# hasindu2008/sigtk

Hardware: AMD Instinct MI355X
Metric: event_raw_samples_per_sec (higher is better)
Workload: dtype f32+f64; 1 GPU; sigtk event (DNA params) on 10000 synthetic reads x 100000 samples per GPU (BASELINE configs[1]), device-resident; reads_per_gpu=10000, samples_per_read=100000, samples_per_gpu=1000000000, fallback_reads=0, rerun_chunks=0, long_detector_replays=66843, long_detector_replay_indices=87526, split_reads=0, batches_in_flight=1, parallelism=reads sharded across ranks, no collective

## Files before the change

sigtk_amd/csrc/event_detect.h:

```cpp
#pragma once
#include <utility>

#include "event_device.h"

namespace sgk {

template <int W1>
struct LzCfg {
    static constexpr int W2 = 2 * W1;
    static constexpr int R = 16;
    static constexpr int NP = (W1 == 3) ? 8 : 16;
    static constexpr int NA = (W1 == 3) ? 4 : 8;
    static constexpr int NL = (W1 == 3) ? 8 : 16;
    static constexpr int H1 = W1 / 2;
};
static_assert(LzCfg<3>::NP >= 8 && LzCfg<7>::NP >= 16, "prefix ring holds P(i) .. P(i+W2+1)");

#ifndef SGK_EVENT_LEAD
#define SGK_EVENT_LEAD 1
#endif

constexpr int LZ_NONE = -(1 << 29);
constexpr int LZ_NREC = 8;
constexpr int LZ_RING_WORDS = 16;

struct LzSnap {
    LzSnapState init[64];
    LzSnapState at_e[64];
    LzSnapState st0[64];
};
__device__ inline bool lz_equal(const LzSnapState &a, const LzSnapState &b) {
    return a.sp == b.sp && __float_as_int(a.sv) == __float_as_int(b.sv) && a.lm == b.lm && a.r0 == b.r0 &&
           a.bits == b.bits;
}
struct LzLds {
    uint32_t ring[64][LZ_RING_WORDS + 1];
    LzSnap snap;
    LzRun runs[64][LZ_NREC];
    int nrec[64];
};

template <typename T>
__device__ __attribute__((noinline)) float tstat_exact_at(const T *base, Scale sc, int i, int w) {
    double A = 0.0, A2 = 0.0, B = 0.0, B2 = 0.0;
    for (int k = 0; k < w; ++k) {
        const float xa = to_pa(base[i - w + k], sc);
        const float xb = to_pa(base[i + k], sc);
        A = A + (double)xa;
        A2 = A2 + (double)(xa * xa);
        B = B + (double)xb;
        B2 = B2 + (double)(xb * xb);
    }
    if (w == 3) return sgk_tstat_ref<3>(A, A2, B, B2);
    if (w == 6) return sgk_tstat_ref<6>(A, A2, B, B2);
    if (w == 7) return sgk_tstat_ref<7>(A, A2, B, B2);
    return sgk_tstat_ref<14>(A, A2, B, B2);
}

template <typename T>
struct Lead16;
template <>
struct Lead16<int16_t> {
    uint32_t w[8];
    template <int U>
    __device__ __forceinline__ float get(const Scale &sc) const {
        const int v = (U & 1) ? ((int)w[U / 2] >> 16) : (int)(short)(w[U / 2] & 0xffffu);
        const float shifted = (float)v + sc.offf;
        return shifted * sc.unit;
    }
};
template <>
struct Lead16<float> {
    float w[16];
    template <int U>
    __device__ __forceinline__ float get(const Scale &) const { return w[U]; }
};
typedef uint32_t sgk_u32x4_a4 __attribute__((ext_vector_type(4), aligned(4)));

template <typename T>
__device__ __attribute__((noinline)) Lead16<T> lead_fix_head(Lead16<T> g, int pos, T first) {
    T tmp[16];
    __builtin_memcpy(tmp, g.w, sizeof(tmp));
#pragma unroll
    for (int k = 0; k < 16; ++k) tmp[k] = (pos + k < 0) ? first : tmp[k];
    __builtin_memcpy(g.w, tmp, sizeof(tmp));
    return g;
}

constexpr int REP_MAX_EVENTS = 32;
struct RepairCtx {
    const double *P, *P2;
    const int *ev;
    int nev;
    bool all_dirty;
};

__device__ __attribute__((noinline)) float tstat_prefix_at(const double *P, const double *P2, int i, int w) {
    const double p0 = P[i], q0 = P2[i];
    const double A = p0 - P[i - w], A2 = q0 - P2[i - w], B = P[i + w] - p0, B2 = P2[i + w] - q0;
    if (w == 3) return sgk_tstat_ref<3>(A, A2, B, B2);
    if (w == 6) return sgk_tstat_ref<6>(A, A2, B, B2);
    if (w == 7) return sgk_tstat_ref<7>(A, A2, B, B2);
    return sgk_tstat_ref<14>(A, A2, B, B2);
}

template <int W1>
__device__ __forceinline__ void repair_mark(const RepairCtx &rep, int &next_t, int q0, unsigned cnt1, unsigned cnt2,
                                            unsigned &bad1, unsigned &bad2) {
    constexpr int W2 = 2 * W1;
    if (rep.all_dirty) {
#pragma unroll
        for (int u = 0; u < 4; ++u) {
            if ((unsigned)(q0 + u - W1) < cnt1) bad1 |= 1u << u;
            if ((unsigned)(q0 + u - W2) < cnt2) bad2 |= 1u << u;
        }
        return;
    }
    if (next_t > q0 + 3 + W2 - 1) return;
    int nt = 0x7fffffff;
    for (int k = 0; k < rep.nev; ++k) {
        const int t = rep.ev[k];
#pragma unroll
        for (int u = 0; u < 4; ++u) {
            const int i = q0 + u;
            if ((unsigned)(i - t + W1 - 1) < (unsigned)(2 * W1) && (unsigned)(i - W1) < cnt1) bad1 |= 1u << u;
            if ((unsigned)(i - t + W2 - 1) < (unsigned)(2 * W2) && (unsigned)(i - W2) < cnt2) bad2 |= 1u << u;
        }
        if (t + W2 >= q0 + 4 && t < nt) nt = t;
    }
    next_t = nt;
}

constexpr int LZ_PRE = LZ_RING_WORDS;
__device__ __attribute__((noinline)) void lz_emit_slow(uint32_t *ring, unsigned long long *bm, int flushed,
                                                       int i_begin, int s, int e, int p, int cur) {
    const int own_lo = s - i_begin;
    if (p < own_lo) {
        if (cur >= own_lo) ring[LZ_PRE] = (uint32_t)(i_begin + p);
        return;
    }
    if (p >= flushed) {
        atomicOr(&ring[(p >> 5) & (LZ_RING_WORDS - 1)], 1u << (p & 31));
    } else {
        const int pa = i_begin + p;
        if (pa >= s && pa < e) atomicOr(reinterpret_cast<uint32_t *>(bm) + (pa >> 5), 1u << (pa & 31));
    }
}
__device__ __attribute__((noinline)) int lz_record(LzRun *runs, int nrec, int a, int b, int s, int e, int n) {
    if ((b >= s && b < e) || (b == n && e == n && s < n)) {
        if (nrec < LZ_NREC) {
            runs[nrec].a = a;
            runs[nrec].b = b;
        }
        ++nrec;
    }
    return nrec;
}

struct Redo4 {
    float v[4];
};
template <int W1, typename T, bool FLAGGED>
__device__ __attribute__((noinline)) Redo4 redo_quad(const T *base, Scale sc, const double *P, const double *P2, int i0,
                                                     unsigned cnt1, unsigned bits, float t0, float t1, float t2,
                                                     float t3) {
    Redo4 r;
    r.v[0] = t0; r.v[1] = t1; r.v[2] = t2; r.v[3] = t3;
#pragma unroll
    for (int k = 0; k < 4; ++k) {
        if ((bits >> k) & 1u) {
            const int i = i0 + k;
            float v = 0.0f;
            if ((unsigned)(i - W1) < cnt1) {
                if constexpr (FLAGGED) v = tstat_prefix_at(P, P2, i, W1);
                else v = tstat_exact_at<T>(base, sc, i, W1);
            }
            r.v[k] = v;
        }
    }
    return r;
}

typedef unsigned long long lmask_t;
__device__ __forceinline__ bool lane_of(lmask_t m) { return __builtin_amdgcn_inverse_ballot_w64(m); }

template <int W1, typename T, bool FLAGGED, bool LEAD = false>
struct LazyPass {
    static_assert(!(LEAD && FLAGGED), "the fallback keeps its domain checks and TwoSum form");
    using C = LzCfg<W1>;
    static constexpr int W2 = C::W2, R = C::R, NP = C::NP, NA = C::NA, NL = C::NL, H1 = C::H1;
    static constexpr int NA2 = LEAD ? 2 * NA : NA;
    static constexpr int NS = LEAD ? NA : 1;
    static_assert(NA2 > (LEAD ? 2 : 1) * W1 && (!LEAD || NS > W1) && R % NA2 == 0, "ring depths");
    double Ps[NP], Pq[NP];
    SgkARole ar[NA2];
    float ss[NS], sqs[NS];
    SgkLSide ls[NL];
    float t1[4];
    lmask_t nk[4];
    lmask_t hc[4];
    Lead16<T> cur;
    float sv;
    int sp;
    lmask_t inpk, val, strong;
    lmask_t hist[H1 + 1];
    uint32_t bw;
    int lm, r0;
    lmask_t hot;
    int nrec;
    uint32_t *ring;
    LzRun *runs;
    const T *base;
    int lo, hi;
    Scale sc;
    int n, s, e, i_begin, ib, jb, flushed;
    unsigned cnt1, cnt2;
    lmask_t done;
    bool slow;
    bool oldpeak;
    unsigned long long *bm;
    RepairCtx rep;
    int next_t;
    int dirty;

    __device__ __forceinline__ void load_lead(Lead16<T> &dst, int pos) const {
        int p = pos > hi - 16 ? hi - 16 : pos;
        p = p < lo ? lo : p;
        constexpr int NV = 16 * (int)sizeof(T) / 16;
        const sgk_u32x4_a4 *src = reinterpret_cast<const sgk_u32x4_a4 *>(base + p);
        sgk_u32x4_a4 v[NV];
#pragma unroll
        for (int k = 0; k < NV; ++k) v[k] = src[k];
        __builtin_memcpy(dst.w, v, sizeof(dst.w));
        if (pos < 0) dst = lead_fix_head<T>(dst, pos, base[0]);
    }

    template <int U>
    __device__ __forceinline__ void tstep() {
        const float xn = cur.template get<U>(sc);
        const float xqn = xn * xn;
        Ps[(U + W2 + 1) % NP] = Ps[(U + W2) % NP] + (double)xn;
        Pq[(U + W2 + 1) % NP] = Pq[(U + W2) % NP] + (double)xqn;
        if constexpr (LEAD) {
            const double c = Ps[(U + W2) % NP] - Ps[(U + W1) % NP], cq = Pq[(U + W2) % NP] - Pq[(U + W1) % NP];
            const float s_p = (float)c, sq_p = (float)cq;
            const float s_i = ss[U % NS], sq_i = sqs[U % NS];
            ss[(U + W1) % NS] = s_p;
            sqs[(U + W1) % NS] = sq_p;
            bool cv_ok, tail_ok;
            t1[U & 3] = sgk_tstat_try_ab<W1>(s_i, sq_i, ar[(U + NA2 - W1) % NA2], cv_ok, tail_ok);
            nk[U & 3] = ~(__ballot(cv_ok) & __ballot(tail_ok));
            ar[(U + W1) % NA2] = sgk_arole<W1, true>(c, cq);
            const SgkLSide lb = sgk_lside_halves<W2>(s_i, sq_i, s_p, sq_p);
            hc[U & 3] = ~__ballot(sgk_long_cold<W2>(ls[(U + NL - W2) % NL], lb));
            ls[U % NL] = lb;
            return;
        }
        const double p0 = Ps[U % NP], q0 = Pq[U % NP];
        const double b1 = Ps[(U + W1) % NP] - p0, b1q = Pq[(U + W1) % NP] - q0;
        const double b2 = Ps[(U + W2) % NP] - p0, b2q = Pq[(U + W2) % NP] - q0;
        const SgkLSide lb = sgk_lside<W2>(b2, b2q);
        if constexpr (!FLAGGED) {
            bool cv_ok, tail_ok;
            t1[U & 3] = sgk_tstat_try_ab<W1>(b1, b1q, ar[(U + NA - W1) % NA], cv_ok, tail_ok);
            nk[U & 3] = ~(__ballot(cv_ok) & __ballot(tail_ok));
            ar[U % NA] = sgk_arole<W1, true>(b1, b1q);
            hc[U & 3] = ~__ballot(sgk_long_cold<W2>(ls[(U + NL - W2) % NL], lb));
            ls[U % NL] = lb;
        } else {
            bool ok;
            const float v = sgk_tstat_try_ab<W1>(b1, b1q, ar[(U + NA - W1) % NA], ok);
            ok = ok && sgk_try_domain<W1>(b1, b1q, ar[(U + NA - W1) % NA]);
            const double a_s = Ps[(U + W2) % NP], b_s = (double)xn, r_s = Ps[(U + W2 + 1) % NP];
            const double a_q = Pq[(U + W2) % NP], b_q = (double)xqn, r_q = Pq[(U + W2 + 1) % NP];
            const double t_s = r_s - a_s, t_q = r_q - a_q;
            const double e_s = (a_s - (r_s - t_s)) + (b_s - t_s), e_q = (a_q - (r_q - t_q)) + (b_q - t_q);
            const bool clean = U > dirty;
            if (e_s != 0.0 || e_q != 0.0) dirty = dirty > U + 2 * W2 ? dirty : U + 2 * W2;
            ok = ok && clean;
            ar[U % NA] = sgk_arole<W1, false>(b1, b1q);
            bool cold = sgk_long_cold<W2>(ls[(U + NL - W2) % NL], lb);
            cold = cold && clean && sgk_lside_domain(ls[(U + NL - W2) % NL]) && sgk_lside_domain(lb);
            ls[U % NL] = lb;
            t1[U & 3] = v;
            nk[U & 3] = ~__ballot(ok);
            hc[U & 3] = ~__ballot(cold);
        }
    }

    template <bool SLOW>
    __device__ __forceinline__ void dstep_core(const int u, const float v, const lmask_t hck, const lmask_t live) {
        constexpr float ph = DetParam<W1>::ph, thr1 = DetParam<W1>::thr1;
        const float d1 = v - sv;
        const float ee = lane_of(inpk) ? d1 : -d1;
        lmask_t P = __ballot(ee > 0.0f);
        lmask_t Q = __ballot(ee < -ph);
        const lmask_t Tt = __ballot(v > thr1);
        if constexpr (SLOW) {
            P &= live;
            Q &= live;
        }
        const lmask_t ent = Q & ~inpk;
        const lmask_t pos = (inpk & P) | ent;
        strong = (pos & Tt) | (strong & ~pos);
        lmask_t dom = inpk & strong;
        if constexpr (SLOW) dom &= live;
        val = inpk & (val | (Q & strong));
        lmask_t recent = hist[0];
#pragma unroll
        for (int k = 1; k < H1; ++k) recent |= hist[k];
        lmask_t em = val & ~P & ~recent;
        if constexpr (SLOW) em &= live;
        const lmask_t upd = P | ent | em;
        const uint32_t bit = 1u << ((jb + u - H1 - 1) & 31);
        if (SLOW && oldpeak) {
            if (lane_of(em)) {
                lz_emit_slow(ring, bm, flushed, i_begin, s, e, jb + sp, jb + u);
                lm = sp;
                r0 = u;
            }
        } else {
            if (lane_of(em)) {
                bw |= bit;
                lm = sp;
                r0 = u;
            }
            const lmask_t erare = em & ~hist[H1];
            if (erare != 0ull) {
                if (lane_of(erare)) {
                    bw &= ~bit;
                    const int p = jb + sp, own = s - i_begin;
                    if (p >= own) atomicOr(&ring[(p >> 5) & (LZ_RING_WORDS - 1)], 1u << (p & 31));
                    else if (jb >= own) ring[LZ_PRE] = (uint32_t)(i_begin + p);
                }
            }
        }
        sv = lane_of(upd) ? v : sv;
        sp = lane_of(pos) ? u : sp;
        inpk = (inpk & ~em) | ent;
        val = val & ~em;
        if constexpr (SLOW) {
#pragma unroll
            for (int k = H1; k >= 1; --k) hist[k] = (hist[k - 1] & live) | (hist[k] & ~live);
            hist[0] = pos | (hist[0] & ~live);
        } else {
#pragma unroll
            for (int k = H1; k >= 1; --k) hist[k] = hist[k - 1];
            hist[0] = pos;
        }
        const lmask_t rec = dom & hot;
        if (rec != 0ull) {
            if (lane_of(rec)) nrec = lz_record(runs, nrec, ib + max(r0, lm + W1 + 1), ib + u, s, e, n);
        }
        lmask_t on = __ballot(lm < u - W1);
        if constexpr (SLOW) on &= live;
        hot = (hot & ~dom) | (on & hck & (~dom | em));
    }
    __device__ __forceinline__ void bw_advance() {
        const int p = jb - 1;
        atomicOr(&ring[(p >> 5) & (LZ_RING_WORDS - 1)], bw);
        bw = 0u;
    }
    template <int U>
    __device__ __forceinline__ void dstep() {
        if constexpr (U == H1 + 1) {
            if ((jb & 16) == 0) bw_advance();
        }
        dstep_core<false>(U, t1[U & 3], hc[U & 3], ~0ull);
    }
    template <int U>
    __device__ __forceinline__ void dstep_edge() {
        if constexpr (U == H1 + 1) {
            if ((jb & 16) == 0) bw_advance();
        }
        const lmask_t live = ~done & __ballot((unsigned)(ib + U) < (unsigned)n);
        dstep_core<true>(U, t1[U & 3], hc[U & 3], live);
    }
    __device__ __forceinline__ void slow_fix(const int u0) {
#pragma unroll
        for (int k = 0; k < 4; ++k) {
            const bool in1 = (unsigned)(ib + u0 + k - W1) < cnt1;
            t1[k] = in1 ? t1[k] : 0.0f;
            nk[k] &= __ballot(in1);
            hc[k] &= __ballot((unsigned)(ib + u0 + k - W2) < cnt2);
        }
    }

    template <int U0>
    __device__ __forceinline__ void quad() {
        tstep<U0>();
        tstep<U0 + 1>();
        tstep<U0 + 2>();
        tstep<U0 + 3>();
        if (slow) slow_fix(U0);
        if constexpr (FLAGGED) {
            unsigned bad1 = 0u, bad2 = 0u;
            repair_mark<W1>(rep, next_t, ib + U0, cnt1, cnt2, bad1, bad2);
#pragma unroll
            for (int k = 0; k < 4; ++k) {
                nk[k] |= __ballot(((bad1 >> k) & 1u) != 0u);
                hc[k] |= __ballot(((bad2 >> k) & 1u) != 0u);
            }
        }
        const lmask_t anybad = (nk[0] | nk[1] | nk[2] | nk[3]) & ~done;
        if (anybad != 0ull) {
            if (lane_of(anybad)) {
                const unsigned bits = (lane_of(nk[0]) ? 1u : 0u) | (lane_of(nk[1]) ? 2u : 0u) |
                                      (lane_of(nk[2]) ? 4u : 0u) | (lane_of(nk[3]) ? 8u : 0u);
                const Redo4 r4 = redo_quad<W1, T, FLAGGED>(base, sc, rep.P, rep.P2, ib + U0, cnt1, bits, t1[0], t1[1],
                                                           t1[2], t1[3]);
                t1[0] = r4.v[0]; t1[1] = r4.v[1]; t1[2] = r4.v[2]; t1[3] = r4.v[3];
            }
        }
        if (slow) {
            dstep_edge<U0>();
            dstep_edge<U0 + 1>();
            dstep_edge<U0 + 2>();
            dstep_edge<U0 + 3>();
        } else {
            dstep<U0>();
            dstep<U0 + 1>();
            dstep<U0 + 2>();
            dstep<U0 + 3>();
        }
    }

    template <int K>
    __device__ __forceinline__ void init_step(double &ps, double &pq, const float (&w)[2 * W2], double (&hs)[W2 + 1],
                                              double (&hq)[W2 + 1]) {
        const float x = w[K];
        ps = ps + (double)x;
        pq = pq + (double)(x * x);
        constexpr int k1 = K + 1;
        if constexpr (k1 <= W2) { hs[k1] = ps; hq[k1] = pq; }
        if constexpr (k1 >= W2) { Ps[(k1 - W2) % NP] = ps; Pq[(k1 - W2) % NP] = pq; }
        if constexpr (k1 >= W2 && k1 < W2 + W1) {
            constexpr int pr = k1 - W1;
            ar[((k1 - W1 - W2) % NA + NA) % NA] = sgk_arole<W1, !FLAGGED>(ps - hs[pr], pq - hq[pr]);
        }
        if constexpr (k1 >= W2 && k1 < 2 * W2) {
            constexpr int pr = k1 - W2;
            ls[((k1 - 2 * W2) % NL + NL) % NL] = sgk_lside<W2>(ps - hs[pr], pq - hq[pr]);
        }
    }
    template <int... Ks>
    __device__ __forceinline__ void init_rings(const float (&w)[2 * W2], std::integer_sequence<int, Ks...>) {
        double ps = 0.0, pq = 0.0;
        double hs[W2 + 1], hq[W2 + 1];
        hs[0] = 0.0;
        hq[0] = 0.0;
        (init_step<Ks>(ps, pq, w, hs, hq), ...);
    }

    __device__ __forceinline__ void init_lead(const float (&w)[2 * W2]) {
        double hs[2 * W2 + 1], hq[2 * W2 + 1];
        hs[0] = 0.0;
        hq[0] = 0.0;
#pragma unroll
        for (int k = 0; k < 2 * W2; ++k) {
            hs[k + 1] = hs[k] + (double)w[k];
            hq[k + 1] = hq[k] + (double)(w[k] * w[k]);
        }
#pragma unroll
        for (int k = W2; k <= 2 * W2; ++k) { Ps[(k - W2) % NP] = hs[k]; Pq[(k - W2) % NP] = hq[k]; }
        float sf[W2 + W1], sqf[W2 + W1];
#pragma unroll
        for (int j = 0; j < W2 + W1; ++j) {
            const double c = hs[j + W1] - hs[j], cq = hq[j + W1] - hq[j];
            sf[j] = (float)c;
            sqf[j] = (float)cq;
            if (j >= W1) ar[(j - W2 + NA2) % NA2] = sgk_arole<W1, true>(c, cq);
            if (j >= W2) { ss[(j - W2) % NS] = sf[j]; sqs[(j - W2) % NS] = sqf[j]; }
        }
#pragma unroll
        for (int j = 0; j < W2; ++j) ls[(j - W2 + NL) % NL] = sgk_lside_halves<W2>(sf[j], sqf[j], sf[j + W1], sqf[j + W1]);
    }

    template <int... Qs>
    __device__ __forceinline__ void block(std::integer_sequence<int, Qs...>) {
        (quad<4 * Qs>(), ...);
    }
};

__device__ __forceinline__ void lz_flush(uint32_t *ring, unsigned long long *bm, int i_begin, int p0, int own_lo,
                                         int own_hi) {
    uint16_t *bm16 = reinterpret_cast<uint16_t *>(bm);
#pragma unroll
    for (int k = 0; k < 8; ++k) {
        const int p = p0 + 32 * k;
        const int wi = (p >> 5) & (LZ_RING_WORDS - 1);
        const uint32_t w = ring[wi];
        ring[wi] = 0u;
        if (p >= own_lo && p < own_hi) bm16[(i_begin + p) >> 4] = (uint16_t)(w & 0xffffu);
        if (p + 16 >= own_lo && p + 16 < own_hi) bm16[(i_begin + p + 16) >> 4] = (uint16_t)(w >> 16);
    }
}

template <int W1, typename T, bool FLAGGED, bool LEAD = false>
__device__ __forceinline__ void pass_lazy(const ReadCtx<T> &rc, bool given, int lead, int steps, bool active, int s,
                                          int e, LzLds *L, const RepairCtx *rep, bool by_progress = false) {
    using LP = LazyPass<W1, T, FLAGGED, LEAD>;
    constexpr int W2 = LP::W2, R = LP::R;
    if (!__any(active)) return;
    const int l = lane_id();
    LP f;
    f.n = (int)rc.n;
    f.s = active ? s : 0x7fffffff;
    f.e = active ? e : 0x7fffffff;
    f.bm = rc.bm;
    f.sc = rc.sc;
    f.base = rc.base;
    f.lo = (int)(rc.lo < -(1 << 30) ? -(1 << 30) : rc.lo);
    f.hi = (int)(rc.hi > 0x7fffffffLL ? 0x7fffffffLL : rc.hi);
    f.ring = L->ring[l];
    f.runs = L->runs[l];
    const int n = f.n;
    const int i_begin = s - lead;
    f.i_begin = i_begin;
#pragma unroll
    for (int k = 0; k < LZ_RING_WORDS; ++k) f.ring[k] = 0u;
    if (active) f.ring[LZ_PRE] = 0xffffffffu;
#pragma unroll
    for (int k = 0; k < 4; ++k) { f.t1[k] = 0.0f; f.nk[k] = 0ull; f.hc[k] = 0ull; }
    {
        float w[2 * W2];
#pragma unroll
        for (int k = 0; k < 2 * W2; ++k) {
            int p = i_begin - W2 + k;
            p = p > f.hi - 1 ? f.hi - 1 : p;
            p = p < 0 ? 0 : p;
            w[k] = to_pa(f.base[p], f.sc);
        }
#pragma unroll
        for (int k = 0; k < LP::NP; ++k) { f.Ps[k] = 0.0; f.Pq[k] = 0.0; }
        if constexpr (LEAD) f.init_lead(w);
        else f.init_rings(w, std::make_integer_sequence<int, 2 * W2>{});
        if (i_begin == 0) {
            if constexpr (LEAD) {
#pragma unroll
                for (int k = 1; k <= W1; ++k) f.ar[LP::NA2 - k].va = __builtin_nan("");
            } else {
#pragma unroll
                for (int k = 0; k < LP::NA; ++k) f.ar[k].va = __builtin_nan("");
            }
        }
    }
    f.load_lead(f.cur, i_begin + W2);

    f.sv = FLT_MAX;
    f.sp = 0;
    f.inpk = 0ull; f.val = 0ull; f.strong = 0ull; f.hot = 0ull;
#pragma unroll
    for (int k = 0; k <= LP::H1; ++k) f.hist[k] = 0ull;
    f.bw = 0u;
    f.lm = LZ_NONE;
    f.r0 = 0;
    if (__any(given)) {
        LzSnapState st = L->snap.st0[l];
        if (!given) { st.sp = -1; st.sv = FLT_MAX; st.lm = LZ_NONE; st.r0 = i_begin; st.bits = 0u; }
        f.sv = st.sv;
        f.inpk = __ballot((st.bits & 1u) != 0u);
        f.val = __ballot((st.bits & 2u) != 0u);
        f.strong = __ballot((st.bits & 4u) != 0u);
        f.hot = __ballot((st.bits & 8u) != 0u);
        f.sp = (st.bits & 1u) ? st.sp - i_begin : 0;
        f.lm = st.lm == LZ_NONE ? LZ_NONE : st.lm - W1 - i_begin;
#pragma unroll
        for (int k = 0; k <= LP::H1; ++k) f.hist[k] = __ballot((st.bits & 1u) && st.sp == i_begin - 1 - k);
        f.r0 = st.r0 - i_begin;
    }
    f.nrec = 0;
    f.done = ~__ballot(active);
    f.flushed = 0;
    if constexpr (FLAGGED) {
        f.dirty = 2 * W2;
        f.rep = *rep;
        f.next_t = 0x7fffffff;
        for (int k = 0; k < f.rep.nev; ++k) {
            const int t = f.rep.ev[k];
            if (t + W2 >= i_begin && t < f.next_t) f.next_t = t;
        }
    }
    const int main_steps = steps;
    f.cnt1 = (n - 2 * W1 + 1) > 0 ? (unsigned)(n - 2 * W1 + 1) : 0u;
    f.cnt2 = (n - 2 * W2 + 1) > 0 ? (unsigned)(n - 2 * W2 + 1) : 0u;
    const int own_lo = lead, own_hi = active ? lead + (e - s) : lead;

    auto snapshot = [&](int ib) -> LzSnapState {
        LzSnapState st;
        const bool ip = lane_of(f.inpk);
        st.sv = f.sv;
        st.sp = ip ? ib + f.sp : -1;
        st.lm = (f.lm + W1 < 0) ? LZ_NONE : ib + f.lm + W1;
        st.r0 = ib + max(f.r0, f.lm + W1 + 1);
        st.bits = (ip ? 1u : 0u) | ((ip && lane_of(f.val)) ? 2u : 0u) | ((ip && lane_of(f.strong)) ? 4u : 0u) |
                  (lane_of(f.hot) ? 8u : 0u);
        return st;
    };

    constexpr int PRIO_STEPS = 400;
    const int q1 = by_progress ? main_steps - 3 * PRIO_STEPS : -1, q2 = by_progress ? main_steps - 2 * PRIO_STEPS : -1,
              q3 = by_progress ? main_steps - PRIO_STEPS : -1;
    if (by_progress) {
        if (q1 > 0) __builtin_amdgcn_s_setprio(3);
        else if (q2 > 0) __builtin_amdgcn_s_setprio(2);
        else if (q3 > 0) __builtin_amdgcn_s_setprio(1);
        else __builtin_amdgcn_s_setprio(0);
    }
    int jb = 0;
    for (;;) {
        const int ib = i_begin + jb;
        if ((jb & 255) == 0 && jb >= 512) {
            lz_flush(f.ring, f.bm, i_begin, jb - 512, own_lo, own_hi);
            f.flushed = jb - 256;
        }
        const bool lane_edge = ib + R - 1 > n - W2;
        const lmask_t old_peak = __ballot(f.sp < -(256 - 2 * R)) | (__ballot(f.sp + jb < own_lo) & __ballot(jb == own_lo));
        f.oldpeak = (old_peak & f.inpk & ~f.done) != 0ull;
        f.slow = f.oldpeak || (__ballot(lane_edge) & ~f.done) != 0ull;
        f.ib = ib;
        f.jb = jb;
        Lead16<T> nxt;
        f.load_lead(nxt, ib + R + W2);
        f.block(std::make_integer_sequence<int, R / 4>{});
        f.cur = nxt;
        f.sp -= R;
        f.lm = f.lm < LZ_NONE ? LZ_NONE : f.lm - R;
        f.r0 -= R;
        if constexpr (FLAGGED) f.dirty = f.dirty < -(1 << 20) ? f.dirty : f.dirty - R;
        jb += R;
        if (jb == q1) __builtin_amdgcn_s_setprio(2);
        else if (jb == q2) __builtin_amdgcn_s_setprio(1);
        else if (jb == q3) __builtin_amdgcn_s_setprio(0);
        {
            const int nb = i_begin + jb;
            if (active && lead > 0 && jb == lead) L->snap.init[l] = snapshot(nb);
            if (active && nb == e) L->snap.at_e[l] = snapshot(nb);
            const lmask_t reach = __ballot(nb >= e) & ~f.done;
            if ((reach & f.hot) != 0ull) {
                if (lane_of(reach & f.hot) && e == n) f.nrec = lz_record(f.runs, f.nrec, nb + max(f.r0, f.lm + W1 + 1), n, s, e, n);
            }
            f.done |= reach;
            f.inpk &= ~reach;
            f.val &= ~reach;
            f.strong &= ~reach;
        }
        if (jb >= main_steps && f.done == ~0ull) break;
    }
    {
        const int p = jb - LP::H1 - 2 < 0 ? 0 : jb - LP::H1 - 2;
        atomicOr(&f.ring[(p >> 5) & (LZ_RING_WORDS - 1)], f.bw);
    }
    for (int p0 = f.flushed; p0 < jb; p0 += 256) lz_flush(f.ring, f.bm, i_begin, p0, own_lo, own_hi);
    if (active) L->nrec[l] = f.nrec;
}

template <int W1, typename T, bool FLAGGED, bool COLLECT = false>
__device__ inline void replay_run(const ReadCtx<T> &rc, const RepairCtx *rep, bool has, int i, int b, int bits_lo,
                           int bits_hi, EvHeader *hdr, int *found = nullptr) {
    if (has && b > i) atomicAdd(&hdr->n_replay_idx, (unsigned long long)(b - i));
    constexpr int W2 = 2 * W1;
    constexpr float ph = DetParam<W1>::ph, thr2 = DetParam<W1>::thr2;
    const int n = (int)rc.n;
    const unsigned cnt2 = (n - 2 * W2 + 1) > 0 ? (unsigned)(n - 2 * W2 + 1) : 0u;
    uint32_t *bm32 = reinterpret_cast<uint32_t *>(rc.bm);
    int lp = -1;
    float lv = FLT_MAX;
    bool lvalid = false;
    while (__any(has && i < b)) {
        if (has && i < b) {
            float v2 = 0.0f;
            if ((unsigned)(i - W2) < cnt2) {
                if constexpr (FLAGGED) v2 = tstat_prefix_at(rep->P, rep->P2, i, W2);
                else v2 = tstat_exact_at<T>(rc.base, rc.sc, i, W2);
            }
            if (lp < 0) {
                if (v2 < lv) {
                    lv = v2;
                } else if (v2 - lv > ph) {
                    lv = v2;
                    lp = i;
                }
            } else {
                if (v2 > lv) {
                    lv = v2;
                    lp = i;
                }
                if (lv - v2 > ph && lv > thr2) lvalid = true;
                if (lvalid && (i - lp) > W2 / 2) {
                    if (lp > 0 && lp < n && lp >= bits_lo && lp < bits_hi) {
                        if constexpr (COLLECT) *found = 1;
                        else atomicOr(&bm32[lp >> 5], 1u << (lp & 31));
                    }
                    lp = -1;
                    lv = v2;
                    lvalid = false;
                }
            }
            ++i;
        }
    }
}
template <int W1, typename T, bool FLAGGED>
__device__ void replay_long_runs(const ReadCtx<T> &rc, LzLds *L, const RepairCtx *rep, bool active, int bits_lo,
                                 EvHeader *hdr) {
    const int l = lane_id();
    const int nrec = active ? L->nrec[l] : 0;
    for (int k = 0; k < LZ_NREC; ++k) {
        const bool has = k < nrec;
        if (!__any(has)) break;
        const int i = has ? L->runs[l][k].a : 0;
        const int b = has ? L->runs[l][k].b : 0;
        replay_run<W1, T, FLAGGED>(rc, rep, has, i, b, bits_lo, 0x7fffffff, hdr);
    }
}

template <int W1, typename T, bool FLAGGED, bool MULTI = false, bool LEAD = false>
__device__ __forceinline__ int detect_span(const ReadCtx<T> &rc, EvHeader *hdr, LzLds *L, const RepairCtx *rep,
                                           const int a, const int b, const int mode, const int lead_override,
                                           SegState *seg, const int lanes = 64) {
    const int n = (int)rc.n;
    if constexpr (!MULTI) {
        if (b <= a) return 0;
    }
    const int len = b - a;
    int lead = len < 32768 ? LEAD_DNA_SHORT : LEAD_DNA;
    if (W1 == 7) lead = len <= 32768 ? LEAD_RNA_SHORT : LEAD_RNA;
    if constexpr (MULTI) {
        const long long len64 = (long long)len * (64 / lanes);
        lead = len64 < 32768 ? LEAD_DNA_SHORT : LEAD_DNA;
        if (W1 == 7) lead = len64 <= 32768 ? LEAD_RNA_SHORT : LEAD_RNA;
    }
    if (lead_override > 0) lead = lead_override;
    const bool no_fast = (reinterpret_cast<uintptr_t>(rc.base) & 3u) != 0 || rc.hi < (int64_t)n + 16;
    if constexpr (!MULTI) {
        if (no_fast) return 1;
    }
    const int c = MULTI ? (lane_id() & (lanes - 1)) : lane_id();
    int K, s, e0, lead_c;
    if (mode == 1) {
        K = 16 * ((len + 1023) / 1024);
        s = a + c * K;
        e0 = s + K;
        lead_c = lead;
    } else {
        K = MULTI ? chunk_len_lanes(len, lead, lanes) : chunk_len_fast(len, lead);
        s = c == 0 ? a : a + c * K + lead;
        e0 = c == 0 ? a + lead + K : s + K;
        lead_c = c > 0 ? lead : 0;
    }
    int TT = lead + K;
    int Kmax = K;
    if constexpr (MULTI) {
#pragma unroll
        for (int d = 32; d >= 1; d >>= 1) {
            const int o = __shfl_xor(Kmax, d, 64), t = __shfl_xor(TT, d, 64);
            Kmax = o > Kmax ? o : Kmax;
            TT = t > TT ? t : TT;
        }
    }
    const int e = e0 < b ? e0 : b;
    const bool active = s < b && !(MULTI && no_fast);
    {
        LzSnapState z;
        z.sp = -1; z.sv = FLT_MAX; z.lm = LZ_NONE; z.r0 = 0; z.bits = 0u;
        L->snap.init[lane_id()] = z;
        L->snap.at_e[lane_id()] = z;
        L->nrec[lane_id()] = 0;
        L->ring[lane_id()][LZ_PRE] = 0xffffffffu;
    }
    bool run = active;
    bool first = true;
    const int l = lane_id();
    const uint32_t pol = FLAGGED ? 0u : prio_policy(rc.dev);
    for (int iter = 0; iter < 66; ++iter) {
        pass_lazy<W1, T, FLAGGED, LEAD>(rc, first ? (mode == 2 && c == 0) : true, first ? lead_c : 0, first ? TT : Kmax, run,
                                        s, e, L, rep, first && (pol == 1u || pol == 2u));
        __syncthreads();
        const LzSnapState pe = L->snap.at_e[c > 0 ? l - 1 : l];
        const LzSnapState mine = L->snap.init[l];
        const bool bad = active && c > 0 && !lz_equal(pe, mine);
        const unsigned long long badmask = __ballot(bad);
        if (badmask == 0ull) break;
        __syncthreads();
        if (bad) {
            L->snap.init[l] = pe;
            L->snap.st0[l] = pe;
        }
        run = bad;
        first = false;
        if (l == 0) atomicAdd(&hdr->n_rerun, (uint32_t)__popcll(badmask));
        __syncthreads();
    }
    int rcode = 0;
    if constexpr (MULTI) {
        const unsigned long long over = __ballot(active && L->nrec[l] > LZ_NREC);
        const unsigned long long grp = (lanes >= 64 ? ~0ull : ((1ull << lanes) - 1ull)) << (l & ~(lanes - 1));
        if (no_fast) rcode = 1;
        else if (over & grp) rcode = 2;
    } else {
        if (__any(active && L->nrec[l] > LZ_NREC)) return 2;
    }
    const bool mine_ok = active && rcode == 0;
    if (seg) {
        const int last = __popcll(__ballot(active)) - 1;
        if (l == 0) {
            seg->init0 = L->snap.init[0];
            seg->end = L->snap.at_e[last];
        }
        const int nrec = active ? L->nrec[l] : 0;
        int ncross = 0;
        for (int k = 0; k < nrec; ++k) ncross += (L->runs[l][k].a < a) ? 1 : 0;
        const int incl = wave_incl_scan_i(ncross);
        const int total = wave_last_i(incl);
        if (total > SEG_CROSS_MAX) rcode = 2;
        else {
            int at = incl - ncross;
            for (int k = 0; k < nrec; ++k) {
                if (L->runs[l][k].a < a) seg->cross[at++] = L->runs[l][k];
            }
        }
        if (l == 0) seg->n_cross = total > SEG_CROSS_MAX ? 0u : (uint32_t)total;
    }
    const int pre = mine_ok ? (int)L->ring[l][LZ_PRE] : -1;
    const bool pre_out = pre >= 0 && pre < a;
    if (seg) {
        const int npre = pre_out ? 1 : 0;
        const int incl = wave_incl_scan_i(npre);
        const int total = wave_last_i(incl);
        if (total > SEG_PRE_MAX) rcode = 2;
        else if (npre) seg->pre[incl - 1] = pre;
        if (l == 0) seg->n_pre = total > SEG_PRE_MAX ? 0u : (uint32_t)total;
    }
    const unsigned long long hotm = __ballot(mine_ok && L->nrec[l] > 0);
    const bool anypre = __any(pre >= 0);
    if (hotm != 0ull || anypre) {
        if (l == 0 && hotm != 0ull) atomicAdd(&hdr->n_hot_runs, (uint32_t)__popcll(hotm));
        __threadfence_block();
        __syncthreads();
        if (pre >= 0 && !pre_out) atomicOr(reinterpret_cast<uint32_t *>(rc.bm) + (pre >> 5), 1u << (pre & 31));
        if (hotm != 0ull) replay_long_runs<W1, T, FLAGGED>(rc, L, rep, mine_ok, a, hdr);
    }
    return rcode;
}
template <int W1, typename T, bool FLAGGED>
__device__ __forceinline__ int detect_read_lazy(const ReadCtx<T> &rc, EvHeader *hdr, LzLds *L, const RepairCtx *rep) {
    const int n = (int)rc.n;
    if (n <= 0) return 0;
    return detect_span<W1, T, FLAGGED>(rc, hdr, L, rep, 0, n, 0, 0, nullptr);
}

}
```

Before: 301.3 billion samples/s.

## Track run-start bookkeeping with wave bitmasks instead of per-step ballot on lm

```diff
diff --git a/sigtk_amd/csrc/event_detect.h b/sigtk_amd/csrc/event_detect.h
--- a/sigtk_amd/csrc/event_detect.h
+++ b/sigtk_amd/csrc/event_detect.h
@@ -20,6 +20,10 @@
 #define SGK_EVENT_LEAD 1
 #endif
 
+#ifndef SGK_EVENT_BOOK
+#define SGK_EVENT_BOOK 1
+#endif
+
 constexpr int LZ_NONE = -(1 << 29);
 constexpr int LZ_NREC = 8;
 constexpr int LZ_RING_WORDS = 16;
@@ -192,6 +196,8 @@
     static constexpr int NA2 = LEAD ? 2 * NA : NA;
     static constexpr int NS = LEAD ? NA : 1;
     static_assert(NA2 > (LEAD ? 2 : 1) * W1 && (!LEAD || NS > W1) && R % NA2 == 0, "ring depths");
+    static constexpr bool BOOK = ((SGK_EVENT_BOOK) & (FLAGGED ? 4 : (LEAD ? 1 : 2))) != 0;
+    static constexpr int NM = W1 - H1;
     double Ps[NP], Pq[NP];
     SgkARole ar[NA2];
     float ss[NS], sqs[NS];
@@ -206,6 +212,8 @@
     lmask_t hist[H1 + 1];
     uint32_t bw;
     int lm, r0;
+    lmask_t moff[NM - 1];
+    int rs;
     lmask_t hot;
     int nrec;
     uint32_t *ring;
@@ -313,17 +321,37 @@
         if constexpr (SLOW) em &= live;
         const lmask_t upd = P | ent | em;
         const uint32_t bit = 1u << ((jb + u - H1 - 1) & 31);
+        lmask_t off = 0ull, nx[NM - 1];
         if (SLOW && oldpeak) {
             if (lane_of(em)) {
                 lz_emit_slow(ring, bm, flushed, i_begin, s, e, jb + sp, jb + u);
-                lm = sp;
-                r0 = u;
+                if constexpr (BOOK) {
+                    rs = max(u, sp + W1 + 1);
+                } else {
+                    lm = sp;
+                    r0 = u;
+                }
+            }
+            if constexpr (BOOK) {
+                off = moff[0];
+#pragma unroll
+                for (int k = 0; k < NM - 1; ++k) nx[k] = k + 1 < NM - 1 ? moff[k + 1] : 0ull;
+                book_mask_from_sp<NM - 1>(em, u, off, nx);
             }
         } else {
-            if (lane_of(em)) {
-                bw |= bit;
-                lm = sp;
-                r0 = u;
+            if constexpr (BOOK) {
+                if (lane_of(em)) bw |= bit;
+                rs = lane_of(em) ? u + NM : rs;
+                const lmask_t eusual = em & hist[H1];
+                off = moff[0] | eusual;
+#pragma unroll
+                for (int k = 0; k < NM - 1; ++k) nx[k] = k + 1 < NM - 1 ? (moff[k + 1] | eusual) : eusual;
+            } else {
+                if (lane_of(em)) {
+                    bw |= bit;
+                    lm = sp;
+                    r0 = u;
+                }
             }
             const lmask_t erare = em & ~hist[H1];
             if (erare != 0ull) {
@@ -332,7 +360,9 @@
                     const int p = jb + sp, own = s - i_begin;
                     if (p >= own) atomicOr(&ring[(p >> 5) & (LZ_RING_WORDS - 1)], 1u << (p & 31));
                     else if (jb >= own) ring[LZ_PRE] = (uint32_t)(i_begin + p);
+                    if constexpr (BOOK) rs = max(u, sp + W1 + 1);
                 }
+                if constexpr (BOOK) book_mask_from_sp<NM - 2>(erare, u, off, nx);
             }
         }
         sv = lane_of(upd) ? v : sv;
@@ -350,11 +380,31 @@
         }
         const lmask_t rec = dom & hot;
         if (rec != 0ull) {
-            if (lane_of(rec)) nrec = lz_record(runs, nrec, ib + max(r0, lm + W1 + 1), ib + u, s, e, n);
-        }
-        lmask_t on = __ballot(lm < u - W1);
+            if (lane_of(rec)) nrec = lz_record(runs, nrec, ib + run_start(), ib + u, s, e, n);
+        }
+        lmask_t on;
+        if constexpr (BOOK) {
+            on = ~off;
+#pragma unroll
+            for (int k = 0; k < NM - 1; ++k) {
+                if constexpr (SLOW) moff[k] = (nx[k] & live) | (moff[k] & ~live);
+                else moff[k] = nx[k];
+            }
+        } else {
+            on = __ballot(lm < u - W1);
+        }
         if constexpr (SLOW) on &= live;
         hot = (hot & ~dom) | (on & hck & (~dom | em));
+    }
+    __device__ __forceinline__ int run_start() const {
+        if constexpr (BOOK) return rs;
+        else return max(r0, lm + W1 + 1);
+    }
+    template <int KN>
+    __device__ __forceinline__ void book_mask_from_sp(const lmask_t m, const int u, lmask_t &off, lmask_t (&nx)[NM - 1]) const {
+        off |= m & __ballot(sp + W1 >= u);
+#pragma unroll
+        for (int k = 0; k < KN; ++k) nx[k] |= m & __ballot(sp + W1 >= u + k + 1);
     }
     __device__ __forceinline__ void bw_advance() {
         const int p = jb - 1;
@@ -555,6 +605,9 @@
     f.bw = 0u;
     f.lm = LZ_NONE;
     f.r0 = 0;
+    f.rs = 0;
+#pragma unroll
+    for (int k = 0; k < LP::NM - 1; ++k) f.moff[k] = 0ull;
     if (__any(given)) {
         LzSnapState st = L->snap.st0[l];
         if (!given) { st.sp = -1; st.sv = FLT_MAX; st.lm = LZ_NONE; st.r0 = i_begin; st.bits = 0u; }
@@ -568,6 +621,12 @@
 #pragma unroll
         for (int k = 0; k <= LP::H1; ++k) f.hist[k] = __ballot((st.bits & 1u) && st.sp == i_begin - 1 - k);
         f.r0 = st.r0 - i_begin;
+        if constexpr (LP::BOOK) {
+            const int mt = st.lm == LZ_NONE ? LZ_NONE : st.lm - i_begin;
+            f.rs = max(st.r0 - i_begin, mt + 1);
+#pragma unroll
+            for (int k = 0; k < LP::NM - 1; ++k) f.moff[k] = __ballot(mt >= k);
+        }
     }
     f.nrec = 0;
     f.done = ~__ballot(active);
@@ -591,8 +650,9 @@
         const bool ip = lane_of(f.inpk);
         st.sv = f.sv;
         st.sp = ip ? ib + f.sp : -1;
-        st.lm = (f.lm + W1 < 0) ? LZ_NONE : ib + f.lm + W1;
-        st.r0 = ib + max(f.r0, f.lm + W1 + 1);
+        if constexpr (LP::BOOK) st.lm = (f.rs - 1 < 0) ? LZ_NONE : ib + f.rs - 1;
+        else st.lm = (f.lm + W1 < 0) ? LZ_NONE : ib + f.lm + W1;
+        st.r0 = ib + f.run_start();
         st.bits = (ip ? 1u : 0u) | ((ip && lane_of(f.val)) ? 2u : 0u) | ((ip && lane_of(f.strong)) ? 4u : 0u) |
                   (lane_of(f.hot) ? 8u : 0u);
         return st;
@@ -625,8 +685,12 @@
         f.block(std::make_integer_sequence<int, R / 4>{});
         f.cur = nxt;
         f.sp -= R;
-        f.lm = f.lm < LZ_NONE ? LZ_NONE : f.lm - R;
-        f.r0 -= R;
+        if constexpr (LP::BOOK) {
+            f.rs -= R;
+        } else {
+            f.lm = f.lm < LZ_NONE ? LZ_NONE : f.lm - R;
+            f.r0 -= R;
+        }
         if constexpr (FLAGGED) f.dirty = f.dirty < -(1 << 20) ? f.dirty : f.dirty - R;
         jb += R;
         if (jb == q1) __builtin_amdgcn_s_setprio(2);
@@ -638,7 +702,7 @@
             if (active && nb == e) L->snap.at_e[l] = snapshot(nb);
             const lmask_t reach = __ballot(nb >= e) & ~f.done;
             if ((reach & f.hot) != 0ull) {
-                if (lane_of(reach & f.hot) && e == n) f.nrec = lz_record(f.runs, f.nrec, nb + max(f.r0, f.lm + W1 + 1), n, s, e, n);
+                if (lane_of(reach & f.hot) && e == n) f.nrec = lz_record(f.runs, f.nrec, nb + f.run_start(), n, s, e, n);
             }
             f.done |= reach;
             f.inpk &= ~reach;
@@ -702,8 +766,8 @@
     }
 }
 template <int W1, typename T, bool FLAGGED>
-__device__ void replay_long_runs(const ReadCtx<T> &rc, LzLds *L, const RepairCtx *rep, bool active, int bits_lo,
-                                 EvHeader *hdr) {
+__device__ inline void replay_long_runs(const ReadCtx<T> &rc, LzLds *L, const RepairCtx *rep, bool active, int bits_lo,
+                                        EvHeader *hdr) {
     const int l = lane_id();
     const int nrec = active ? L->nrec[l] : 0;
     for (int k = 0; k < LZ_NREC; ++k) {
```

Measured after the change: 304.6 billion samples/s, median of 6. 1.1% higher.
